# jithinjosepkl/mpi-perf

Hardware: AMD Instinct MI355X
Metric: per-pair xGMI GB/s at 4 MB + 8 B latency us; all-pairs aggregate GB/s at 2/4/8 GPUs (higher is better)
Workload: dtype u8

## Files before the change

### mpi-perf_amd/csrc/mpx_kernels.hip

```cpp
#include "mpx_internal.h"

namespace mpx {

typedef unsigned int v4u __attribute__((ext_vector_type(4)));

constexpr u64 kGolden = 0x9E3779B97F4A7C15ull;
constexpr int kAuxSys = 17;
constexpr int kAuxSysNt = 19;
constexpr int kAuxSysVol = (int)0x80000011u;
constexpr int kLLUnits = kLLGranules / 2;
constexpr int kLLUnitsPerLane = kLLUnits / kBlock;
constexpr unsigned kRsrcWord3 = 0x00020000;

__device__ __forceinline__ u64 mix64(u64 z) {
    z = (z ^ (z >> 30)) * 0xbf58476d1ce4e5b9ull;
    z = (z ^ (z >> 27)) * 0x94d049bb133111ebull;
    return z ^ (z >> 31);
}
__device__ __forceinline__ u64 csum_term(u64 w, u64 k) { return mix64(w + (k + 1) * kGolden); }
__device__ __forceinline__ u64 fill_word(u64 key, u64 k) { return mix64((key ^ k) + kGolden); }

__device__ __forceinline__ u64 ld_sys(const u64* p) {
    return __hip_atomic_load(p, __ATOMIC_RELAXED, __HIP_MEMORY_SCOPE_SYSTEM);
}
__device__ __forceinline__ void st_sys(u64* p, u64 v) {
    __hip_atomic_store(p, v, __ATOMIC_RELAXED, __HIP_MEMORY_SCOPE_SYSTEM);
}
__device__ __forceinline__ void drain_stores() { asm volatile("s_waitcnt vmcnt(0)" ::: "memory"); }
__device__ __forceinline__ u64 now_ticks() { return __builtin_amdgcn_s_memrealtime(); }

__device__ __forceinline__ __amdgpu_buffer_rsrc_t rsrc(const void* base, unsigned bytes) {
    return __builtin_amdgcn_make_buffer_rsrc(const_cast<void*>(base), 0, (int)bytes, kRsrcWord3);
}

__device__ __forceinline__ u64 block_sum(u64 v, u64* lds4) {
    for (int o = 32; o > 0; o >>= 1) v += __shfl_xor(v, o, 64);
    const int wave = threadIdx.x >> 6;
    if ((threadIdx.x & 63) == 0) lds4[wave] = v;
    __syncthreads();
    u64 s = 0;
    if (threadIdx.x == 0) s = lds4[0] + lds4[1] + lds4[2] + lds4[3];
    __syncthreads();
    return s;
}

template <bool NT>
__device__ __forceinline__ v4u ld16(const v4u* p) {
    if constexpr (NT) return __builtin_nontemporal_load(p);
    else return *p;
}
template <bool NT>
__device__ __forceinline__ void st16(v4u* p, v4u v) {
    if constexpr (NT) __builtin_nontemporal_store(v, p);
    else *p = v;
}

template <int U, bool LDNT, bool STNT, bool CONTIG>
__global__ __launch_bounds__(kBlock) void k_copy(const v4u* __restrict__ src, v4u* __restrict__ dst,
                                                size_t n16, unsigned tail) {
    size_t i, end, stride;
    if constexpr (CONTIG) {
        const size_t per = (n16 + gridDim.x - 1) / gridDim.x;
        const size_t lo = (size_t)blockIdx.x * per;
        end = lo + per < n16 ? lo + per : n16;
        i = lo + threadIdx.x;
        stride = kBlock;
    } else {
        end = n16;
        i = (size_t)blockIdx.x * kBlock + threadIdx.x;
        stride = (size_t)gridDim.x * kBlock;
    }
    for (; i + (U - 1) * stride < end; i += U * stride) {
        v4u r[U];
#pragma unroll
        for (int u = 0; u < U; ++u) r[u] = ld16<LDNT>(src + i + u * stride);
#pragma unroll
        for (int u = 0; u < U; ++u) st16<STNT>(dst + i + u * stride, r[u]);
    }
    for (; i < end; i += stride) st16<STNT>(dst + i, ld16<LDNT>(src + i));
    if (blockIdx.x == 0 && threadIdx.x < tail) {
        const unsigned char* s8 = reinterpret_cast<const unsigned char*>(src + n16);
        unsigned char* d8 = reinterpret_cast<unsigned char*>(dst + n16);
        d8[threadIdx.x] = s8[threadIdx.x];
    }
}

constexpr int kCopyStepsBatch = 8;

template <int T, bool XCD>
__global__ __launch_bounds__(T) void k_copy_steps(const v4u* __restrict__ src, v4u* __restrict__ dst, size_t n16,
                                                 unsigned tail, int iters, u64* bar, int drain, int one_xcd) {
    if (one_xcd && (blockIdx.x & 7)) return;
    const unsigned wg = one_xcd ? blockIdx.x >> 3 : blockIdx.x;
    const u64 g = one_xcd ? gridDim.x >> 3 : gridDim.x;
    const size_t stride = (size_t)g * T;
    const size_t first = (size_t)wg * T + threadIdx.x;
    const int x = (int)(wg & 7);
    const u64 nx = (g - (u64)x + 7) / 8;
    const u64 groups = g < 8 ? g : 8;
    const bool one_unit = n16 <= stride;
    __shared__ int s_stop;
    for (int s = 0; s < iters; ++s) {
        if (one_unit) {
            if (first < n16) __builtin_nontemporal_store(__builtin_nontemporal_load(src + first), dst + first);
        } else for (size_t base = first; base < n16; base += kCopyStepsBatch * stride) {
            v4u r[kCopyStepsBatch];
#pragma unroll
            for (int u = 0; u < kCopyStepsBatch; ++u)
                if (base + u * stride < n16) r[u] = __builtin_nontemporal_load(src + base + u * stride);
#pragma unroll
            for (int u = 0; u < kCopyStepsBatch; ++u)
                if (base + u * stride < n16) __builtin_nontemporal_store(r[u], dst + base + u * stride);
        }
        if (wg == 0 && threadIdx.x < tail) {
            const unsigned char* s8 = reinterpret_cast<const unsigned char*>(src + n16);
            reinterpret_cast<unsigned char*>(dst + n16)[threadIdx.x] = s8[threadIdx.x];
        }
        if (s + 1 == iters) break;
        if (drain) drain_stores();
        __syncthreads();
        if (g == 1) continue;
        if (threadIdx.x == 0) {
            s_stop = 0;
            u64 want;
            if constexpr (XCD) {
                const u64 old = __hip_atomic_fetch_add(bar + 16 * (1 + x), 1ull, __ATOMIC_RELAXED,
                                                       __HIP_MEMORY_SCOPE_AGENT);
                if (old + 1 == nx * (u64)(s + 1))
                    __hip_atomic_fetch_add(bar, 1ull, __ATOMIC_RELAXED, __HIP_MEMORY_SCOPE_AGENT);
                want = groups * (u64)(s + 1);
            } else {
                __hip_atomic_fetch_add(bar, 1ull, __ATOMIC_RELAXED, __HIP_MEMORY_SCOPE_AGENT);
                want = g * (u64)(s + 1);
            }
            const u64 t0 = now_ticks();
            u64 spins = 0;
            while (__hip_atomic_load(bar, __ATOMIC_RELAXED, __HIP_MEMORY_SCOPE_AGENT) < want) {
                if ((++spins & 255) == 0 && now_ticks() - t0 > 100000000ull) {
                    __hip_atomic_store(&bar[1], 1ull, __ATOMIC_RELAXED, __HIP_MEMORY_SCOPE_AGENT);
                    s_stop = 1;
                    break;
                }
                __builtin_amdgcn_s_sleep(1);
            }
        }
        __syncthreads();
        if (s_stop) return;
    }
}

constexpr int kPipeCopyWaves = 4;
constexpr int kPipeThreads = (kPipeCopyWaves + 1) * 64;
constexpr int kAuxNt = 2;


__device__ __forceinline__ void wg_barrier_nofence() {
    asm volatile("s_waitcnt lgkmcnt(0)" ::: "memory");
    __builtin_amdgcn_s_barrier();
    asm volatile("" ::: "memory");
}

template <int UPL>
__global__ __launch_bounds__(kPipeThreads) void k_copy_pipe(const v4u* src, v4u* dst,
                                                          size_t n16, unsigned tail, int iters, u64* bar,
                                                          int hier) {
    __shared__ int s_stop;
    if (threadIdx.x >= kPipeCopyWaves * 64) {
        const unsigned grid = gridDim.x;
        const unsigned g = blockIdx.x & 7;
        const u64 ng = (grid - g + 7) / 8;
        const u64 groups = grid < 8 ? grid : 8;
        for (int s = 0; s + 1 < iters; ++s) {
            wg_barrier_nofence();
            if (threadIdx.x == kPipeCopyWaves * 64) {
                s_stop = 0;
                u64 want;
                const u64* poll;
                if (hier) {
                    const u64 old = __hip_atomic_fetch_add(bar + 16 * (1 + g), 1ull, __ATOMIC_RELAXED,
                                                           __HIP_MEMORY_SCOPE_AGENT);
                    if (old + 1 == ng * (u64)(s + 1)) {
                        const u64 t = __hip_atomic_fetch_add(bar, 1ull, __ATOMIC_RELAXED, __HIP_MEMORY_SCOPE_AGENT);
                        if (t + 1 == groups * (u64)(s + 1))
                            for (u64 k = 0; k < groups; ++k)
                                __hip_atomic_store(bar + 16 * (9 + k), (u64)(s + 1), __ATOMIC_RELAXED,
// ... 50 lines not shown
        return !s_stop;
    };
    load(a, ta);
    for (int s = 0;;) {
        if (s + 1 == iters) { store(a, ta); break; }
        load(b, tb8);
        store(a, ta);
        if (!grid_barrier()) break;
        if (++s + 1 == iters) { store(b, tb8); break; }
        load(a, ta);
        store(b, tb8);
        if (!grid_barrier()) break;
        ++s;
    }
}

__global__ __launch_bounds__(kBlock) void k_fill(unsigned char* p, size_t n, int pattern, u64 arg) {
    const size_t nw = n / 8;
    const size_t stride = (size_t)gridDim.x * kBlock;
    u64* p64 = reinterpret_cast<u64*>(p);
    const u64 bytew = (arg & 0xff) * 0x0101010101010101ull;
    for (size_t k = (size_t)blockIdx.x * kBlock + threadIdx.x; k < nw; k += stride)
        p64[k] = pattern == MPX_FILL_BYTE ? bytew : fill_word(arg, k);
    const unsigned tail = (unsigned)(n & 7);
    if (blockIdx.x == 0 && threadIdx.x < tail) {
        const u64 w = pattern == MPX_FILL_BYTE ? bytew : fill_word(arg, nw);
        p[nw * 8 + threadIdx.x] = (unsigned char)(w >> (8 * threadIdx.x));
    }
}

__device__ __forceinline__ u64 tail_word(const unsigned char* p, size_t off, size_t n) {
    u64 w = 0;
    for (size_t b = 0; off + b < n && b < 8; ++b) w |= (u64)p[off + b] << (8 * b);
    return w;
}

__global__ __launch_bounds__(kBlock) void k_checksum(const unsigned char* p, size_t n, u64* out) {
    __shared__ u64 lds4[4];
    const size_t n16 = n / 16;
    const size_t stride = (size_t)gridDim.x * kBlock;
    const v4u* p16 = reinterpret_cast<const v4u*>(p);
    u64 acc = 0;
    for (size_t v = (size_t)blockIdx.x * kBlock + threadIdx.x; v < n16; v += stride) {
        const v4u x = p16[v];
        acc += csum_term(((u64)x.y << 32) | x.x, 2 * v);
        acc += csum_term(((u64)x.w << 32) | x.z, 2 * v + 1);
    }
    if (blockIdx.x == 0 && threadIdx.x < 2) {
        const size_t off = n16 * 16 + 8 * threadIdx.x;
        if (off < n) acc += csum_term(tail_word(p, off, n), off / 8);
    }
    const u64 s = block_sum(acc, lds4);
    if (threadIdx.x == 0 && s) atomicAdd(out, s);
}

__device__ __forceinline__ u64 rel(const u64* base, u64 v) { return base ? ld_sys(base) + v : v; }

__global__ void k_signal(u64* flag, const u64* base, u64 v) {
    if (threadIdx.x == 0) st_sys(flag, rel(base, v));
}

__global__ void k_wait(const u64* flag, const u64* base, u64 v, Status* st, u64 timeout_ticks) {
    if (threadIdx.x != 0) return;
    if (__hip_atomic_load(&st->err, __ATOMIC_RELAXED, __HIP_MEMORY_SCOPE_SYSTEM)) return;
    const u64 want = rel(base, v);
    const u64 t0 = now_ticks();
    u64 spins = 0, seen;
    while ((seen = ld_sys(flag)) < want) {
        if ((++spins & 255) == 0 && now_ticks() - t0 > timeout_ticks) {
            st->seen = seen;
            st->want = want;
            __hip_atomic_store(&st->err, 1u, __ATOMIC_RELAXED, __HIP_MEMORY_SCOPE_SYSTEM);
            return;
        }
        __builtin_amdgcn_s_sleep(1);
    }
}

__global__ void k_seqbase(u64* base, u64 tx, u64 rx, int add) {
    if (threadIdx.x != 0) return;
    st_sys(base, add ? ld_sys(base) + tx : tx);
    st_sys(base + 1, add ? ld_sys(base + 1) + rx : rx);
}

enum { kTsEntry = 0, kTsPosted = 1, kTsFirst = 2, kTsLoop = 3 };

template <int MODE, bool ANYWG = false>
struct Loop {
    const XferArgs& a;
    int* s_abort;
    u64* lds4;
    v4u* s_tx;
    static constexpr int kUnits = ANYWG ? kLLUnitsPerLane / 2 : kLLUnitsPerLane;
    u64 pre[kUnits];
    u64* s_seen = nullptr;
    mutable bool staged = false;
    mutable u64 ts[4] = {0, 0, 0, 0};
    mutable u64 rdone = 0, rdig = 0;

    __device__ void preload_ll(long long n) {
#pragma unroll
        for (int j = 0; j < kUnits; ++j) {
            const long long off = 8ll * ((int)threadIdx.x + j * kBlock);
            u64 w = 0;
            if (off + 8 <= n) {
                w = *reinterpret_cast<const u64*>(a.tx + off);
            } else {
                for (long long b = 0; off + b < n; ++b) w |= (u64)a.tx[off + b] << (8 * b);
            }
            pre[j] = w;
        }
    }

    __device__ bool aborted() const { return *s_abort != 0; }
    __device__ bool ll_owner() const { return ANYWG || blockIdx.x == 0; }

    __device__ void give_up(int iter) const {
        *s_abort = 1;
        __hip_atomic_store(&a.gbar[1], 1ull, __ATOMIC_RELAXED, __HIP_MEMORY_SCOPE_AGENT);
        __hip_atomic_store(&a.status->where, (unsigned)iter + 1, __ATOMIC_RELAXED, __HIP_MEMORY_SCOPE_SYSTEM);
        __hip_atomic_store(&a.status->err, 1u, __ATOMIC_RELAXED, __HIP_MEMORY_SCOPE_SYSTEM);
    }
    __device__ bool should_stop(u64 spins, u64 t0) const {
        if ((spins & 63) != 0) return false;
        if (*s_abort) return true;
        if (__hip_atomic_load(&a.gbar[1], __ATOMIC_RELAXED, __HIP_MEMORY_SCOPE_AGENT)) return true;
        return now_ticks() - t0 > a.timeout_ticks;
    }

    __device__ bool is_ll(long long n) const { return MODE != MPX_MODE_NONBLOCKING && n <= a.ll_max; }

    __device__ void push_ll(long long n, u64 seq, unsigned goff = 0) const {
        if (!ll_owner()) return;
        const int ng = n > 0 ? (int)((n + 3) >> 2) : 1;
        const int nu = (ng + 1) >> 1;
        const unsigned tag = ll_tag(seq);
        const __amdgpu_buffer_rsrc_t dst = rsrc(&a.peer_mb->ll[a.my_slot][goff], (unsigned)(nu * 16));
#pragma unroll
        for (int j = 0; j < kUnits; ++j) {
            const int u = (int)threadIdx.x + j * kBlock;
            if (u < nu) {
                const v4u v = {(unsigned)pre[j], tag, (unsigned)(pre[j] >> 32), tag};
                __builtin_amdgcn_raw_buffer_store_b128(v, dst, (unsigned)u * 16, 0, kAuxSys);
            }
        }
    }

    __device__ void chunk_of(long long n, long long* lo, long long* hi) const {
        const long long chunk = (((n + a.nwg - 1) / a.nwg) + 15) & ~15ll;
        *lo = (long long)blockIdx.x * chunk;
        *hi = *lo + chunk < n ? *lo + chunk : n;
    }

    template <int AUX, bool STAGE>
    __device__ __forceinline__ void push_units(const v4u* src, __amdgpu_buffer_rsrc_t dst, int nv) const {
        int v = threadIdx.x;
        for (; v + 3 * kBlock < nv; v += 4 * kBlock) {
            const v4u r0 = src[v], r1 = src[v + kBlock], r2 = src[v + 2 * kBlock], r3 = src[v + 3 * kBlock];
            __builtin_amdgcn_raw_buffer_store_b128(r0, dst, v * 16, 0, AUX);
            __builtin_amdgcn_raw_buffer_store_b128(r1, dst, (v + kBlock) * 16, 0, AUX);
            __builtin_amdgcn_raw_buffer_store_b128(r2, dst, (v + 2 * kBlock) * 16, 0, AUX);
            __builtin_amdgcn_raw_buffer_store_b128(r3, dst, (v + 3 * kBlock) * 16, 0, AUX);
            if (STAGE) {
                s_tx[v] = r0;
                s_tx[v + kBlock] = r1;
                s_tx[v + 2 * kBlock] = r2;
                s_tx[v + 3 * kBlock] = r3;
            }
        }
        for (; v < nv; v += kBlock) {
            const v4u r = src[v];
            __builtin_amdgcn_raw_buffer_store_b128(r, dst, v * 16, 0, AUX);
            if (STAGE) s_tx[v] = r;
        }
    }
    template <bool STAGE>
    __device__ __forceinline__ void push_units_aux(const v4u* src, __amdgpu_buffer_rsrc_t dst, int nv) const {
        if (a.stream) push_units<kAuxSysNt, STAGE>(src, dst, nv);
        else push_units<kAuxSys, STAGE>(src, dst, nv);
    }

    __device__ void push_bulk(long long n, u64 seq, bool publish = true, unsigned char* dst_base = nullptr,
                              bool skip = false) const {
        const int w = blockIdx.x;
        if (w >= a.nwg) return;
        long long lo, hi;
        chunk_of(n, &lo, &hi);
        if (lo < hi) {
            const unsigned bytes = (unsigned)(hi - lo);
            const __amdgpu_buffer_rsrc_t dst = rsrc((dst_base ? dst_base : a.peer_rx) + lo, bytes);
            const int nv = (int)(bytes >> 4);
            const v4u* txv = reinterpret_cast<const v4u*>(a.tx + lo);
            if (a.stage && !staged) {
                if (!skip) {
                    push_units_aux<true>(txv, dst, nv);
                } else {
                    for (int v = threadIdx.x; v < nv; v += kBlock) s_tx[v] = txv[v];
                }
            } else if (!skip) {
                push_units_aux<false>(a.stage ? s_tx : txv, dst, nv);
            }
            const unsigned tail = bytes & 15;
            if (threadIdx.x < tail && !skip) {
                const unsigned o = (unsigned)nv * 16 + threadIdx.x;
                __builtin_amdgcn_raw_buffer_store_b8(a.tx[lo + o], dst, o, 0, kAuxSys);
            }
        }
        staged = true;
        if (!publish) return;
        drain_stores();
        __syncthreads();
        if (threadIdx.x == 0) st_sys(&a.peer_mb->flag[a.my_slot][w], seq);
    }

    __device__ void send(long long n, u64 seq, bool skip = false) const {
        if (is_ll(n)) { if (!skip) push_ll(n, seq); else push_ll_tags_only(n, seq); }
        else push_bulk(n, seq, true, nullptr, skip);
    }

    __device__ void push_ll_tags_only(long long n, u64 seq, unsigned goff = 0) const {
        if (!ll_owner()) return;
        const int ng = n > 0 ? (int)((n + 3) >> 2) : 1;
        const int nu = (ng + 1) >> 1;
        const unsigned tag = ll_tag(seq);
        const __amdgpu_buffer_rsrc_t dst = rsrc(&a.peer_mb->ll[a.my_slot][goff], (unsigned)(nu * 16));
        for (int u = threadIdx.x; u < nu; u += kBlock) {
            const v4u v = {~0u, tag, ~0u, tag};
            __builtin_amdgcn_raw_buffer_store_b128(v, dst, (unsigned)u * 16, 0, kAuxSys);
        }
    }

    __device__ bool wait_ll(long long n, u64 seq, int iter, unsigned goff = 0) const {
        const int ng = n > 0 ? (int)((n + 3) >> 2) : 1;
        const int nu = (ng + 1) >> 1;
        const int mine = nu > (int)threadIdx.x ? (nu - (int)threadIdx.x + kBlock - 1) / kBlock : 0;
        const unsigned tag = ll_tag(seq);
        const __amdgpu_buffer_rsrc_t src = rsrc(&a.my_mb->ll[a.peer_slot][goff], (unsigned)(nu * 16));
        v4u x[kUnits];
        if (mine > 0) {
            const u64 t0 = now_ticks();
            u64 spins = 0;
            for (;;) {
#pragma unroll
                for (int j = 0; j < kUnits; ++j)
                    if (j < mine)
                        x[j] = __builtin_amdgcn_raw_buffer_load_b128(src, ((unsigned)threadIdx.x + j * kBlock) * 16, 0,
                                                                     kAuxSysVol);
                bool ok = true;
#pragma unroll
                for (int j = 0; j < kUnits; ++j)
                    if (j < mine) ok &= (x[j].y == tag) & (x[j].w == tag);
                if (ok) break;
                if (should_stop(++spins, t0)) { give_up(iter); break; }
                __builtin_amdgcn_s_sleep(0);
            }
            if (ll_owner() && !*s_abort) {
                const __amdgpu_buffer_rsrc_t rr = rsrc(a.rx, (unsigned)n);
#pragma unroll
                for (int j = 0; j < kUnits; ++j) {
                    if (j >= mine) break;
                    const long long off = 8ll * ((int)threadIdx.x + j * kBlock);
                    const u64 d = ((u64)x[j].z << 32) | x[j].x;
                    if (off + 8 <= n) {
                        const unsigned lo = (unsigned)d, hi = (unsigned)(d >> 32);
                        __builtin_amdgcn_raw_buffer_store_b32(lo, rr, (unsigned)off, 0, kAuxSys);
                        __builtin_amdgcn_raw_buffer_store_b32(hi, rr, (unsigned)off + 4, 0, kAuxSys);
                    } else {
                        for (long long b = 0; off + b < n; ++b)
                            __builtin_amdgcn_raw_buffer_store_b8((unsigned char)(d >> (8 * b)), rr, (unsigned)(off + b),
                                                                 0, kAuxSys);
                    }
                }
            }
        }
        __syncthreads();
        return !aborted();
    }

    __device__ bool wait_bulk(u64 seq, int iter) const {
        if (threadIdx.x < 64) {
            const u64* f = &a.my_mb->flag[a.peer_slot][0];
            const u64 t0 = now_ticks();
            u64 spins = 0;
            for (;;) {
                bool ok = true;
                for (int j = threadIdx.x; j < a.nwg; j += 64) ok &= ld_sys(f + j) >= seq;
                if (__all(ok)) break;
                if (should_stop(++spins, t0)) {
                    if (threadIdx.x == 0) give_up(iter);
                    break;
                }
                __builtin_amdgcn_s_sleep(1);
            }
        }
        __syncthreads();
        return !aborted();
    }

    __device__ bool recv(long long n, u64 seq, int iter) const {
        return is_ll(n) ? wait_ll(n, seq, iter) : wait_bulk(seq, iter);
    }

    __device__ void post_receives() const {
        if (blockIdx.x == 0 && threadIdx.x == 0) st_sys(&a.peer_mb->posted[a.my_slot], a.call);
    }
    __device__ bool peer_posted() const { return ld_sys(&a.my_mb->posted[a.peer_slot]) >= a.call; }
    __device__ bool wait_posted() const {
        if (threadIdx.x == 0) {
            const u64 t0 = now_ticks();
            u64 spins = 0;
            while (!peer_posted()) {
                if (should_stop(++spins, t0)) { give_up(0); break; }
                __builtin_amdgcn_s_sleep(1);
            }
        }
        stamp(kTsPosted);
        __syncthreads();
        return !aborted();
    }

    __device__ void check(long long n, int iter) const {
        const u64 poison = 0x5a5a5a5a5a5a5a5aull ^ (u64)iter;
        const bool last = iter + 1 == a.iters;
        u64 acc = 0;
        if (is_ll(n)) {
            if (ll_owner()) {
                const __amdgpu_buffer_rsrc_t rr = rsrc(a.rx, (unsigned)n);
                for (long long k = threadIdx.x; 8 * k < n; k += kBlock) {
                    const unsigned o = (unsigned)(8 * k);
                    u64 w = 0;
                    if (8 * k + 8 <= n) {
                        w = (u64)__builtin_amdgcn_raw_buffer_load_b32(rr, o, 0, kAuxSys) |
                            ((u64)__builtin_amdgcn_raw_buffer_load_b32(rr, o + 4, 0, kAuxSys) << 32);
                    } else {
                        for (long long b = 0; 8 * k + b < n; ++b)
                            w |= (u64)__builtin_amdgcn_raw_buffer_load_b8(rr, o + (unsigned)b, 0, kAuxSys) << (8 * b);
                    }
                    acc += csum_term(w, k);
                }
                __syncthreads();
                if (!last) {
                    for (long long o = threadIdx.x; o < n; o += kBlock)
                        __builtin_amdgcn_raw_buffer_store_b8((unsigned char)poison, rr, (unsigned)o, 0, kAuxSys);
                    drain_stores();
                }
            }
        } else if ((int)blockIdx.x < a.nwg) {
            acc = sum_chunk(a.rx, n, poison, last);
        }
        const u64 s = block_sum(acc, lds4);
        if (threadIdx.x == 0 && s) atomicAdd(&a.csum[iter], s);
    }

// ... 517 lines not shown
        }
        L.push_bulk(n, a.tx_seq0 + (u64)i + 1, true, L.slot_base(a.peer_rx, a.peer_ring, i), a.skip_push == i + 1);
        if (inflight == kNbWindow - 1) {
            ok = L.nb_wait([&] { return next >= i; }, &next, i);
            if (ok && w == 0) ok = L.nb_waitall(i - inflight, i, &done, &dig, fmix, &next, i);
            inflight = 0;
        } else {
            ++inflight;
        }
    }
    if (ok && inflight > 0) {
        ok = L.nb_wait([&] { return next >= a.iters; }, &next, a.iters - 1);
        if (ok && w == 0) ok = L.nb_waitall(a.iters - inflight, a.iters, &done, &dig, fmix, &next, a.iters - 1);
    }
    if (ok) L.nb_wait([&] { return next >= a.iters; }, &next, a.iters - 1);
    if (w == 0 && threadIdx.x == 0) {
        L.rdone = done;
        L.rdig = dig;
    }
    if (L.last_to_finish()) L.finish_last();
}

template <int MODE, int GROUP, bool LAT>
__device__ __forceinline__ void xfer_pull_body(const XferArgs a) {
    __shared__ int s_abort;
    __shared__ u64 lds4[4];
    __shared__ u64 s_seen;
    if (threadIdx.x == 0) {
        s_abort = 0;
        s_seen = 0;
    }
    Loop<MODE> L{a, &s_abort, lds4, nullptr, {}, &s_seen};
    LatTrace<LAT> T;
    if (!L.wait_go()) {
        if (L.last_to_finish()) L.finish_last();
        return;
    }
    L.stamp(kTsEntry);
    const long long n = a.len;
    const u64 nw = (u64)a.nwg;
    if (MODE == MPX_MODE_UNIDIR && GROUP == 0 && blockIdx.x == 0) L.preload_ll(1);
    __syncthreads();
    u64 txs = a.tx_seq0, rxs = a.rx_seq0, done = 0, pending = 0;
    L.post_receives();
    bool ok = true;
    int inflight = 0;
    if constexpr (LAT) T.begin(a.lat, L.ts[kTsEntry], L.ts[kTsPosted], a.iters);
    for (int i = 0; ok && i < a.iters; ++i) {
        if constexpr (MODE == MPX_MODE_PINGPONG) {
            if constexpr (GROUP == 1) {
                ok = L.pull_send(++txs, nw * (u64)i, i) && L.pull_recv(n, ++rxs, i);
            } else {
                ok = L.pull_recv(n, ++rxs, i) && L.pull_send(++txs, nw * (u64)(i + 1), i);
            }
            if (ok) ++done;
        } else if constexpr (MODE == MPX_MODE_UNIDIR) {
            if constexpr (GROUP == 1) {
                ok = L.pull_send(++txs, 0, i) && L.recv(1, ++rxs, i);
                if (ok) {
                    ++done;
                    if (a.check) L.check(1, i);
                }
            } else {
                ok = L.pull_recv(n, ++rxs, i);
                if (ok) ++done;
                if (ok && blockIdx.x == 0) ok = L.template poll_ge<false>(&a.gbar[kScrLanded], nw * (u64)(i + 1), i);
                if (ok) L.send(1, ++txs);
            }
        } else {
            ++pending;
            const bool pub = (i + 1) % a.nb_publish == 0 || i + 1 == a.iters;
            ok = L.pull_send(++txs, 0, i) && L.pull_recv(n, ++rxs, i, pub ? pending : 0);
            if (pub) pending = 0;
            if (ok && inflight == kNbWindow - 1) {
                ok = L.template poll_ge<false>(&a.gbar[kScrLanded], nw * (u64)(i + 1), i) && L.wait_pulled(txs - 1, i);
                done += (u64)inflight;
                inflight = 0;
            } else {
                ++inflight;
            }
        }
        if constexpr (LAT) {
            if (ok && T.on()) {
                const u64 t = T.tick(i);
                if (i == 0) L.ts[kTsFirst] = t;
            }
        }
    }
    if constexpr (LAT) L.stamp(kTsLoop);
    const bool sent_bulk = MODE != MPX_MODE_UNIDIR || GROUP == 1;
    if (ok && sent_bulk && a.iters > 0 && !a.no_pull_wait) ok = L.wait_pulled(txs, a.iters - 1);
    if constexpr (MODE == MPX_MODE_NONBLOCKING) {
        if (blockIdx.x == 0) {
            if (ok && a.iters > 0) ok = L.template poll_ge<false>(&a.gbar[kScrLanded], nw * (u64)a.iters, a.iters - 1);
            if (ok) done += (u64)inflight;
            u64 part = 0;
            if (ok && a.check) {
                const u64 fmix = mix64((u64)n);
                for (int j = threadIdx.x; j < a.iters; j += kBlock)
                    if (j % kNbWindow != kNbWindow - 1)
                        part += __hip_atomic_load(&a.csum[j], __ATOMIC_RELAXED, __HIP_MEMORY_SCOPE_AGENT) ^ fmix;
            }
            const u64 s = block_sum(part, lds4);
            if (threadIdx.x == 0) {
                L.rdone = done;
                L.rdig = s;
            }
        }
        if (L.last_to_finish()) L.finish_last();
    } else if (L.last_to_finish()) {
        L.account(done, (MODE == MPX_MODE_UNIDIR && GROUP == 1) ? 1 : n);
        if constexpr (LAT) T.end();
        L.finish_last();
    }
}
template <int MODE, int GROUP>
__global__ __launch_bounds__(kBlock, 4) void k_xfer_pull(XferArgs a) {
    xfer_pull_body<MODE, GROUP, false>(a);
}
template <int MODE, int GROUP>
__global__ __launch_bounds__(kBlock, 4) void k_xfer_pull_lat(XferArgs a) {
    xfer_pull_body<MODE, GROUP, true>(a);
}

template <bool CHECK>
__global__ __launch_bounds__(kBlock, 4) __attribute__((amdgpu_num_sgpr(80))) void k_xfer_fan(FanArgs f) {
    __shared__ int s_abort;
    __shared__ u64 lds4[4];
    if (threadIdx.x == 0) s_abort = 0;
    XferArgs x{};
    x.status = f.status;
    x.gbar = f.gbar;
    x.timeout_ticks = f.timeout_ticks;
    x.done_token = f.done_token;
    x.stream = f.stream;
    x.iters = f.iters;
    Loop<MPX_MODE_NONBLOCKING> L{x, &s_abort, lds4, nullptr, {}};
    __syncthreads();
    L.stamp(kTsEntry);
    const unsigned m = f.tab->map[blockIdx.x];
    const int k = (int)(m >> 16), w = (int)(m & 0xffffu);
    FanLink& lk = f.tab->link[k];
    const long long n = f.len;
    const int nw = lk.nwg;
    const u64 tx0 = lk.tx_seq0, rx0 = lk.rx_seq0;
    const long long chunk = (((n + nw - 1) / nw) + 15) & ~15ll;
    const long long lo = (long long)w * chunk;
    const long long hi = lo + chunk < n ? lo + chunk : n;
    const unsigned bytes = lo < hi ? (unsigned)(hi - lo) : 0u;
    const int nv = (int)(bytes >> 4);
    const unsigned tail = bytes & 15;
    const long long at = bytes ? lk.off + lo : 0;
    const unsigned char* src = f.tx + at;
    const __amdgpu_buffer_rsrc_t dst = rsrc(lk.peer_rx + (bytes ? lo : 0), bytes);
    const __amdgpu_buffer_rsrc_t mine = rsrc(f.rx + at, bytes);
    u64* flag_out = &lk.peer_mb->flag[f.my_slot][w];
    u64* credit_out = &lk.peer_mb->credit[f.my_slot][w];
    const u64* flag_in = &f.my_mb->flag[lk.peer][w];
    const u64* credit_in = &f.my_mb->credit[lk.peer][w];

    auto wait_ge = [&](const u64* p, u64 want, int iter) -> bool {
        if (threadIdx.x == 0) {
            const u64 t0 = now_ticks();
            u64 spins = 0;
            while (ld_sys(p) < want) {
                if (L.should_stop(++spins, t0)) { L.give_up(iter); break; }
                __builtin_amdgcn_s_sleep(1);
            }
        }
        __syncthreads();
        return !L.aborted();
    };

    if (w == 0 && threadIdx.x == 0) st_sys(&lk.peer_mb->posted[f.my_slot], lk.call);
    bool ok = f.iters == 0 || wait_ge(&f.my_mb->posted[lk.peer], lk.call, 0);
    L.stamp(kTsPosted);
    u64 done = 0;
    for (int i = 0; ok && i < f.iters; ++i) {
        if (CHECK && i > 0) {
            ok = wait_ge(credit_in, tx0 + (u64)i, i);
            if (!ok) break;
        }
        if (bytes && f.skip_push != i + 1) {
            L.push_units_aux<false>(reinterpret_cast<const v4u*>(src), dst, nv);
            if (threadIdx.x < tail) {
                const unsigned o = (unsigned)nv * 16 + threadIdx.x;
                __builtin_amdgcn_raw_buffer_store_b8(src[o], dst, o, 0, kAuxSys);
            }
        }
        if (CHECK || (i + 1) % f.nb_publish == 0 || i + 1 == f.iters) {
            drain_stores();
            __syncthreads();
            if (threadIdx.x == 0) st_sys(flag_out, tx0 + (u64)i + 1);
        }
        if constexpr (CHECK) {
        ok = wait_ge(flag_in, rx0 + (u64)i + 1, i);
        if (!ok) break;
        const bool keep = i + 1 == f.iters;
        const u64 poison = 0x5a5a5a5a5a5a5a5aull ^ (u64)i;
        u64 acc = 0;
        if (threadIdx.x == 0) __builtin_amdgcn_fence(__ATOMIC_ACQUIRE, "");
        drain_stores();
        __syncthreads();
        if (bytes) {
            const v4u pv = {(unsigned)poison, (unsigned)(poison >> 32), (unsigned)poison, (unsigned)(poison >> 32)};
            for (int v = threadIdx.x; v < nv; v += kBlock) {
                const v4u q = __builtin_amdgcn_raw_buffer_load_b128(mine, v * 16, 0, kAuxSys);
                const u64 kw = (u64)(lo / 8) + 2 * (u64)v;
                acc += csum_term(((u64)q.y << 32) | q.x, kw);
                acc += csum_term(((u64)q.w << 32) | q.z, kw + 1);
                if (!keep) __builtin_amdgcn_raw_buffer_store_b128(pv, mine, v * 16, 0, kAuxSys);
            }
            if (threadIdx.x < 2 && 8 * threadIdx.x < tail) {
                const unsigned o = (unsigned)nv * 16 + 8 * threadIdx.x;
                u64 word = 0;
                for (unsigned b = 0; b < 8 && o + b < bytes; ++b)
                    word |= (u64)__builtin_amdgcn_raw_buffer_load_b8(mine, o + b, 0, kAuxSys) << (8 * b);
                acc += csum_term(word, (u64)(lo + o) / 8);
            }
            __syncthreads();
            if (!keep && threadIdx.x < tail)
                __builtin_amdgcn_raw_buffer_store_b8((unsigned char)poison, mine, (unsigned)nv * 16 + threadIdx.x, 0,
                                                     kAuxSys);
        }
        drain_stores();
        const u64 s = block_sum(acc, lds4);
        if (threadIdx.x == 0) {
            if (s) atomicAdd(&f.csum[lk.csum0 + i], s);
            st_sys(credit_out, rx0 + (u64)i + 1);
        }
        ++done;
        }
    }
    L.stamp(kTsLoop);
    if (!CHECK && ok && f.iters > 0 && wait_ge(flag_in, rx0 + (u64)f.iters, f.iters - 1)) done = (u64)f.iters;
    drain_stores();
    __syncthreads();
    if (threadIdx.x == 0) {
        __hip_atomic_fetch_min(&lk.recv_done, done, __ATOMIC_RELAXED, __HIP_MEMORY_SCOPE_AGENT);
        __hip_atomic_fetch_max(&lk.t_end, now_ticks(), __ATOMIC_RELAXED, __HIP_MEMORY_SCOPE_AGENT);
    }
    if (!L.last_to_finish()) return;
    u64 part = 0, dpart = 0;
    for (int j = threadIdx.x; j < f.nlinks; j += kBlock)
        part += __hip_atomic_load(&f.tab->link[j].recv_done, __ATOMIC_RELAXED, __HIP_MEMORY_SCOPE_AGENT);
    if (CHECK && !__hip_atomic_load(&f.gbar[kScrAbort], __ATOMIC_RELAXED, __HIP_MEMORY_SCOPE_AGENT)) {
        const u64 fmix = mix64((u64)n);
        for (int j = threadIdx.x; j < f.nlinks * f.iters; j += kBlock)
            dpart += __hip_atomic_load(&f.csum[j], __ATOMIC_RELAXED, __HIP_MEMORY_SCOPE_AGENT) ^ fmix;
    }
    const u64 d = block_sum(part, lds4);
    const u64 g = block_sum(dpart, lds4);
    if (threadIdx.x == 0) {
        L.rdone = d;
        L.rdig = g;
    }
    L.finish_last();
}

template <bool CHECK>
__global__ __launch_bounds__(kBlock, 4) __attribute__((amdgpu_num_sgpr(80))) void k_xfer_fan_ll(FanLLArgs q) {
    __shared__ int s_abort;
    __shared__ u64 lds4[4];
    if (threadIdx.x == 0) s_abort = 0;
    const FanArgs& f = q.f;
    const int k = (int)blockIdx.x;
    FanLink& lk = f.tab->link[k];
    const long long n = f.len;
    XferArgs x{};
    x.tx = f.tx + lk.off;
    x.rx = f.rx + lk.off;
    x.my_mb = f.my_mb;
    x.peer_mb = lk.peer_mb;
    x.my_slot = f.my_slot;
    x.peer_slot = lk.peer;
    x.status = f.status;
    x.gbar = f.gbar;
    x.csum = f.csum + lk.csum0;
    x.timeout_ticks = f.timeout_ticks;
    x.done_token = f.done_token;
    x.iters = f.iters;
    x.ll_max = MPX_FAN_LL_MAX;
    Loop<MPX_MODE_PINGPONG, true> L{x, &s_abort, lds4, nullptr, {}};
    __syncthreads();
    L.stamp(kTsEntry);
    const u64 tx0 = lk.tx_seq0, rx0 = lk.rx_seq0;
    if (threadIdx.x == 0) st_sys(&lk.peer_mb->posted[f.my_slot], lk.call);
    L.preload_ll(n);
    bool ok = f.iters > 0;
    if (ok) {
        if (threadIdx.x == 0) {
            const u64 t0 = now_ticks();
            u64 spins = 0;
            while (ld_sys(&f.my_mb->posted[lk.peer]) < lk.call) {
                if (L.should_stop(++spins, t0)) { L.give_up(0); break; }
                __builtin_amdgcn_s_sleep(1);
            }
        }
        __syncthreads();
        ok = !L.aborted();
    }
    L.stamp(kTsPosted);
    u64 done = 0;
    for (int i = 0; ok && i < f.iters; ++i) {
        const u64 s = tx0 + (u64)i + 1, r = rx0 + (u64)i + 1;
        const unsigned out = (unsigned)(s & 1) * kFanLLHalf, in = (unsigned)(r & 1) * kFanLLHalf;
        if (f.skip_push == i + 1) L.push_ll_tags_only(n, s, out);
        else L.push_ll(n, s, out);
        if (q.lag_ticks && k == q.lag_link && i == f.iters / 2) {
            if (threadIdx.x == 0) {
                const u64 t0 = now_ticks();
                while (now_ticks() - t0 < q.lag_ticks) __builtin_amdgcn_s_sleep(127);
            }
            __syncthreads();
        }
        ok = L.wait_ll(n, r, i, in);
        if (!ok) break;
        ++done;
        if constexpr (CHECK) L.check(n, i);
    }
    L.stamp(kTsLoop);
    drain_stores();
    __syncthreads();
    if (threadIdx.x == 0) {
        __hip_atomic_fetch_min(&lk.recv_done, done, __ATOMIC_RELAXED, __HIP_MEMORY_SCOPE_AGENT);
        __hip_atomic_fetch_max(&lk.t_end, now_ticks(), __ATOMIC_RELAXED, __HIP_MEMORY_SCOPE_AGENT);
    }
    if (!L.last_to_finish()) return;
    u64 part = 0, dpart = 0;
    for (int j = threadIdx.x; j < f.nlinks; j += kBlock)
        part += __hip_atomic_load(&f.tab->link[j].recv_done, __ATOMIC_RELAXED, __HIP_MEMORY_SCOPE_AGENT);
    if (CHECK && !__hip_atomic_load(&f.gbar[kScrAbort], __ATOMIC_RELAXED, __HIP_MEMORY_SCOPE_AGENT)) {
        const u64 fmix = mix64((u64)n);
        for (int j = threadIdx.x; j < f.nlinks * f.iters; j += kBlock)
            dpart += __hip_atomic_load(&f.csum[j], __ATOMIC_RELAXED, __HIP_MEMORY_SCOPE_AGENT) ^ fmix;
    }
    const u64 d = block_sum(part, lds4);
    const u64 g = block_sum(dpart, lds4);
    if (threadIdx.x == 0) {
        L.rdone = d;
        L.rdig = g;
    }
    L.finish_last();
}

template <bool CHECK>
__global__ __launch_bounds__(kBlock, 4) __attribute__((amdgpu_num_sgpr(80))) void k_xfer_fan_ll_lat(FanLLArgs q) {
    __shared__ int s_abort;
    __shared__ u64 lds4[4];
    if (threadIdx.x == 0) s_abort = 0;
    const FanArgs& f = q.f;
    const int k = (int)blockIdx.x;
    FanLink& lk = f.tab->link[k];
    const long long n = f.len;
    XferArgs x{};
    x.tx = f.tx + lk.off;
    x.rx = f.rx + lk.off;
    x.my_mb = f.my_mb;
    x.peer_mb = lk.peer_mb;
    x.my_slot = f.my_slot;
    x.peer_slot = lk.peer;
    x.status = f.status;
    x.gbar = f.gbar;
    x.csum = f.csum + lk.csum0;
    x.timeout_ticks = f.timeout_ticks;
    x.done_token = f.done_token;
    x.iters = f.iters;
    x.ll_max = MPX_FAN_LL_MAX;
    Loop<MPX_MODE_PINGPONG, true> L{x, &s_abort, lds4, nullptr, {}};
    __syncthreads();
    L.stamp(kTsEntry);
    const u64 tx0 = lk.tx_seq0, rx0 = lk.rx_seq0;
    if (threadIdx.x == 0) st_sys(&lk.peer_mb->posted[f.my_slot], lk.call);
    L.preload_ll(n);
    bool ok = f.iters > 0;
    if (ok) {
        if (threadIdx.x == 0) {
            const u64 t0 = now_ticks();
            u64 spins = 0;
            while (ld_sys(&f.my_mb->posted[lk.peer]) < lk.call) {
                if (L.should_stop(++spins, t0)) { L.give_up(0); break; }
                __builtin_amdgcn_s_sleep(1);
// ... 253 lines not shown
```

Before: 3237.

## Software-pipeline push copy with double-buffered buffer loads at configurable depth

Rewrites the bulk push loop as a double-buffered pipeline. Each lane issues D raw buffer loads for the next set while storing the previous set to the peer, with separate depths for the pair and fan-out paths. Pointers are made wave-uniform so scalar buffer resources can be built, the LDS-staged resend gets its own store loop, and the flag/credit stores are made explicitly global address space. The aim is more loads in flight to hide source-read latency over xGMI. The cost is higher register pressure, and the last set relies on buffer range clamping for out-of-range lanes.

```diff
diff --git a/mpi-perf_amd/csrc/mpx_kernels.hip b/mpi-perf_amd/csrc/mpx_kernels.hip
--- a/mpi-perf_amd/csrc/mpx_kernels.hip
+++ b/mpi-perf_amd/csrc/mpx_kernels.hip
@@ -11,6 +11,14 @@
 constexpr int kLLUnits = kLLGranules / 2;
 constexpr int kLLUnitsPerLane = kLLUnits / kBlock;
 constexpr unsigned kRsrcWord3 = 0x00020000;
+#ifndef MPX_PUSH_DEPTH_PAIR
+#define MPX_PUSH_DEPTH_PAIR 4
+#endif
+#ifndef MPX_PUSH_DEPTH_FAN
+#define MPX_PUSH_DEPTH_FAN 8
+#endif
+constexpr int kPushDepthPair = MPX_PUSH_DEPTH_PAIR;
+constexpr int kPushDepthFan = MPX_PUSH_DEPTH_FAN;
 
 __device__ __forceinline__ u64 mix64(u64 z) {
     z = (z ^ (z >> 30)) * 0xbf58476d1ce4e5b9ull;
@@ -26,11 +34,23 @@
 __device__ __forceinline__ void st_sys(u64* p, u64 v) {
     __hip_atomic_store(p, v, __ATOMIC_RELAXED, __HIP_MEMORY_SCOPE_SYSTEM);
 }
+typedef __attribute__((address_space(1))) u64 global_u64;
+__device__ __forceinline__ void st_sys_global(u64* p, u64 v) {
+    __hip_atomic_store((global_u64*)p, v, __ATOMIC_RELAXED, __HIP_MEMORY_SCOPE_SYSTEM);
+}
 __device__ __forceinline__ void drain_stores() { asm volatile("s_waitcnt vmcnt(0)" ::: "memory"); }
 __device__ __forceinline__ u64 now_ticks() { return __builtin_amdgcn_s_memrealtime(); }
 
 __device__ __forceinline__ __amdgpu_buffer_rsrc_t rsrc(const void* base, unsigned bytes) {
     return __builtin_amdgcn_make_buffer_rsrc(const_cast<void*>(base), 0, (int)bytes, kRsrcWord3);
+}
+
+template <class T>
+__device__ __forceinline__ T* uniform_ptr(T* p) {
+    const u64 x = (u64)p;
+    const unsigned lo = __builtin_amdgcn_readfirstlane((unsigned)x);
+    const unsigned hi = __builtin_amdgcn_readfirstlane((unsigned)(x >> 32));
+    return reinterpret_cast<T*>(((u64)hi << 32) | lo);
 }
 
 __device__ __forceinline__ u64 block_sum(u64 v, u64* lds4) {
@@ -387,32 +407,63 @@
         *hi = *lo + chunk < n ? *lo + chunk : n;
     }
 
-    template <int AUX, bool STAGE>
-    __device__ __forceinline__ void push_units(const v4u* src, __amdgpu_buffer_rsrc_t dst, int nv) const {
+    template <int AUX, bool STAGE, int D>
+    __device__ __forceinline__ void push_units(const v4u* src, unsigned char* dstp, int nv) const {
+        constexpr unsigned kSet = (unsigned)D * kBlock * 16u;
+        nv = __builtin_amdgcn_readfirstlane(nv);
+        const int nsets = (nv + D * kBlock - 1) / (D * kBlock);
+        if (nsets == 0) return;
+        const unsigned body = (unsigned)nv * 16u;
+        const __amdgpu_buffer_rsrc_t rs = rsrc(uniform_ptr(src), body), rd = rsrc(uniform_ptr(dstp), body);
+        v4u ra[D], rb[D];
+        auto load = [&](v4u (&r)[D], unsigned o) {
+            asm volatile("" ::: "memory");
+#pragma unroll
+            for (int j = 0; j < D; ++j)
+                r[j] = __builtin_amdgcn_raw_buffer_load_b128(rs, o + (unsigned)j * kBlock * 16u, 0, 0);
+        };
+        auto store = [&](v4u (&r)[D], unsigned o) {
+#pragma unroll
+            for (int j = 0; j < D; ++j)
+                __builtin_amdgcn_raw_buffer_store_b128(r[j], rd, o + (unsigned)j * kBlock * 16u, 0, AUX);
+            if (STAGE) {
+#pragma unroll
+                for (int j = 0; j < D; ++j) {
+                    const int v = (int)(o >> 4) + j * kBlock;
+                    if (v < nv) s_tx[v] = r[j];
+                }
+            }
+        };
+        unsigned o = threadIdx.x * 16u;
+        load(ra, o);
+        for (int s = 0;;) {
+            if (s + 1 == nsets) { store(ra, o); break; }
+            load(rb, o + kSet);
+            store(ra, o);
+            o += kSet;
+            if (++s + 1 == nsets) { store(rb, o); break; }
+            load(ra, o + kSet);
+            store(rb, o);
+            o += kSet;
+            ++s;
+        }
+    }
+    template <bool STAGE, int D>
+    __device__ __forceinline__ void push_units_aux(const v4u* src, unsigned char* dstp, int nv) const {
+        if (a.stream) push_units<kAuxSysNt, STAGE, D>(src, dstp, nv);
+        else push_units<kAuxSys, STAGE, D>(src, dstp, nv);
+    }
+    template <int AUX>
+    __device__ __forceinline__ void push_units_lds(__amdgpu_buffer_rsrc_t dst, int nv) const {
         int v = threadIdx.x;
         for (; v + 3 * kBlock < nv; v += 4 * kBlock) {
-            const v4u r0 = src[v], r1 = src[v + kBlock], r2 = src[v + 2 * kBlock], r3 = src[v + 3 * kBlock];
+            const v4u r0 = s_tx[v], r1 = s_tx[v + kBlock], r2 = s_tx[v + 2 * kBlock], r3 = s_tx[v + 3 * kBlock];
             __builtin_amdgcn_raw_buffer_store_b128(r0, dst, v * 16, 0, AUX);
             __builtin_amdgcn_raw_buffer_store_b128(r1, dst, (v + kBlock) * 16, 0, AUX);
             __builtin_amdgcn_raw_buffer_store_b128(r2, dst, (v + 2 * kBlock) * 16, 0, AUX);
             __builtin_amdgcn_raw_buffer_store_b128(r3, dst, (v + 3 * kBlock) * 16, 0, AUX);
-            if (STAGE) {
-                s_tx[v] = r0;
-                s_tx[v + kBlock] = r1;
-                s_tx[v + 2 * kBlock] = r2;
-                s_tx[v + 3 * kBlock] = r3;
-            }
-        }
-        for (; v < nv; v += kBlock) {
-            const v4u r = src[v];
-            __builtin_amdgcn_raw_buffer_store_b128(r, dst, v * 16, 0, AUX);
-            if (STAGE) s_tx[v] = r;
-        }
-    }
-    template <bool STAGE>
-    __device__ __forceinline__ void push_units_aux(const v4u* src, __amdgpu_buffer_rsrc_t dst, int nv) const {
-        if (a.stream) push_units<kAuxSysNt, STAGE>(src, dst, nv);
-        else push_units<kAuxSys, STAGE>(src, dst, nv);
+        }
+        for (; v < nv; v += kBlock) __builtin_amdgcn_raw_buffer_store_b128(s_tx[v], dst, v * 16, 0, AUX);
     }
 
     __device__ void push_bulk(long long n, u64 seq, bool publish = true, unsigned char* dst_base = nullptr,
@@ -423,17 +474,20 @@
         chunk_of(n, &lo, &hi);
         if (lo < hi) {
             const unsigned bytes = (unsigned)(hi - lo);
-            const __amdgpu_buffer_rsrc_t dst = rsrc((dst_base ? dst_base : a.peer_rx) + lo, bytes);
+            unsigned char* dstp = (dst_base ? dst_base : a.peer_rx) + lo;
+            const __amdgpu_buffer_rsrc_t dst = rsrc(dstp, bytes);
             const int nv = (int)(bytes >> 4);
             const v4u* txv = reinterpret_cast<const v4u*>(a.tx + lo);
             if (a.stage && !staged) {
                 if (!skip) {
-                    push_units_aux<true>(txv, dst, nv);
+                    push_units_aux<true, kPushDepthPair>(txv, dstp, nv);
                 } else {
                     for (int v = threadIdx.x; v < nv; v += kBlock) s_tx[v] = txv[v];
                 }
             } else if (!skip) {
-                push_units_aux<false>(a.stage ? s_tx : txv, dst, nv);
+                if (!a.stage) push_units_aux<false, kPushDepthPair>(txv, dstp, nv);
+                else if (a.stream) push_units_lds<kAuxSysNt>(dst, nv);
+                else push_units_lds<kAuxSys>(dst, nv);
             }
             const unsigned tail = bytes & 15;
             if (threadIdx.x < tail && !skip) {
@@ -1257,7 +1311,8 @@
     const unsigned tail = bytes & 15;
     const long long at = bytes ? lk.off + lo : 0;
     const unsigned char* src = f.tx + at;
-    const __amdgpu_buffer_rsrc_t dst = rsrc(lk.peer_rx + (bytes ? lo : 0), bytes);
+    unsigned char* dst_p = lk.peer_rx + (bytes ? lo : 0);
+    const __amdgpu_buffer_rsrc_t dst = rsrc(dst_p, bytes);
     const __amdgpu_buffer_rsrc_t mine = rsrc(f.rx + at, bytes);
     u64* flag_out = &lk.peer_mb->flag[f.my_slot][w];
     u64* credit_out = &lk.peer_mb->credit[f.my_slot][w];
@@ -1277,7 +1332,7 @@
         return !L.aborted();
     };
 
-    if (w == 0 && threadIdx.x == 0) st_sys(&lk.peer_mb->posted[f.my_slot], lk.call);
+    if (w == 0 && threadIdx.x == 0) st_sys_global(&lk.peer_mb->posted[f.my_slot], lk.call);
     bool ok = f.iters == 0 || wait_ge(&f.my_mb->posted[lk.peer], lk.call, 0);
     L.stamp(kTsPosted);
     u64 done = 0;
@@ -1287,7 +1342,7 @@
             if (!ok) break;
         }
         if (bytes && f.skip_push != i + 1) {
-            L.push_units_aux<false>(reinterpret_cast<const v4u*>(src), dst, nv);
+            L.template push_units_aux<false, kPushDepthFan>(reinterpret_cast<const v4u*>(src), dst_p, nv);
             if (threadIdx.x < tail) {
                 const unsigned o = (unsigned)nv * 16 + threadIdx.x;
                 __builtin_amdgcn_raw_buffer_store_b8(src[o], dst, o, 0, kAuxSys);
@@ -1296,7 +1351,7 @@
         if (CHECK || (i + 1) % f.nb_publish == 0 || i + 1 == f.iters) {
             drain_stores();
             __syncthreads();
-            if (threadIdx.x == 0) st_sys(flag_out, tx0 + (u64)i + 1);
+            if (threadIdx.x == 0) st_sys_global(flag_out, tx0 + (u64)i + 1);
         }
         if constexpr (CHECK) {
         ok = wait_ge(flag_in, rx0 + (u64)i + 1, i);
@@ -1332,7 +1387,7 @@
         const u64 s = block_sum(acc, lds4);
         if (threadIdx.x == 0) {
             if (s) atomicAdd(&f.csum[lk.csum0 + i], s);
-            st_sys(credit_out, rx0 + (u64)i + 1);
+            st_sys_global(credit_out, rx0 + (u64)i + 1);
         }
         ++done;
         }
```

Result: no change. 3238 (median of 4 runs) (+0.0%).
